# Nico59000/Ternary-image-codec

Measured on AMD Instinct MI355X. Metric: Mpix/s encode+decode 8K RS(26,20), higher is better.
Workload: dtype u8

## Files before the change

include/t3hip.h:

```cpp
#ifndef T3HIP_H
#define T3HIP_H

#include <stddef.h>
#include <stdint.h>

#ifdef __cplusplus
extern "C" {
#endif

#define T3_OK            0
#define T3_E_NODEVICE   -1
#define T3_E_HIP        -2
#define T3_E_ARG        -3
#define T3_E_CAPACITY   -4
#define T3_E_HEADER     -5
#define T3_E_RS         -6
#define T3_E_COMM       -7

#define T3_P1_RS26_24     0
#define T3_P2_RS26_22     1
#define T3_P3_RS26_20     2
#define T3_P4_RS26_18     3
#define T3_P5_RS26_22_2D  4
#define T3_RAW_MODE       0xFF
// ... 37 lines not shown
typedef struct t3_frame_record {
    uint64_t frame_idx;
    uint64_t n_words;
    uint64_t byte_offset;
    uint32_t crc32;
    uint32_t sym_sum;
    uint8_t  header_syms[54];
    uint8_t  profile;
    uint8_t  mode;
    uint8_t  pad_[8];
} t3_frame_record;

typedef struct t3hip_ctx t3hip_ctx;
int         t3hip_device_count(void);
int         t3hip_init(int device);
int         t3hip_shutdown(void);
int         t3hip_is_ready(void);
int         t3hip_create(int device, t3hip_ctx** out);
int         t3hip_destroy(t3hip_ctx* ctx);
int         t3hip_use(t3hip_ctx* ctx);
t3hip_ctx*  t3hip_current(void);
int         t3hip_ctx_device(const t3hip_ctx* ctx);
const char* t3hip_strerror(int code);
const char* t3hip_last_hip_error(void);
const char* t3hip_version(void);

void t3hip_cfg_default(t3_cfg* cfg);
int  t3hip_plan(uint64_t n_raw_words, const t3_cfg* cfg, t3_layout* out);
uint64_t t3hip_encoded_words(uint64_t n_raw_words, const t3_cfg* cfg);
int  t3hip_gf27_tables(uint8_t* exp78, int16_t* log27, uint8_t* mul729, uint8_t* inv27);
int  t3hip_rs_generator(int k, uint8_t* g_out);
int  t3hip_rs_parity_matrix(int k, int mode, uint8_t* P_out);
int  t3hip_mfma_encode_tables(int k, int mode, uint32_t* afrag768, uint32_t* lds_img3168);
int  t3hip_header_pack(const t3_cfg* cfg, uint32_t frame_seq, uint32_t band_map_hash, uint8_t syms27[27]);
int  t3hip_header_check(const uint8_t syms27[27]);
int  t3hip_header_unpack(const uint8_t syms27[27], t3_cfg* out, uint32_t* frame_seq, uint32_t* band_map_hash);
int  t3hip_header_encode(const t3_cfg* cfg, uint64_t n_raw_words, uint8_t* syms_out, uint32_t* n_syms);

int t3hip_pack_pixels(const void* px6, uint64_t n_px, void* words9);
int t3hip_unpack_words(const void* words9, uint64_t n_words, void* px6);
int t3hip_encode_profile(const void* raw9, uint64_t n_raw, const t3_cfg* cfg,
                         void* out9, uint64_t cap_words, uint64_t* n_out);
int t3hip_decode_profile(const void* in9, uint64_t n_in, t3_cfg* seen,
                         void* out9, uint64_t cap_words, uint64_t* n_out);
int t3hip_encode_frame(const void* px6, uint64_t n_px, const t3_cfg* cfg,
                       void* out9, uint64_t cap_words, uint64_t* n_out);
int t3hip_decode_frame(const void* in9, uint64_t n_in, t3_cfg* seen,
                       void* px6, uint64_t cap_px, uint64_t* n_px);

int t3hip_pack_pixels_dev(const void* d_px6, uint64_t n_px, void* d_words9, void* stream);
int t3hip_unpack_words_dev(const void* d_words9, uint64_t n_words, void* d_px6, void* stream);
int t3hip_encode_profile_dev(const void* d_raw9, uint64_t n_raw, const t3_cfg* cfg,
                             void* d_out9, uint64_t cap_words, uint64_t* n_out, void* stream);
int t3hip_encode_frame_dev(const void* d_px6, uint64_t n_px, const t3_cfg* cfg,
                           void* d_out9, uint64_t cap_words, uint64_t* n_out, void* stream);
int t3hip_decode_profile_dev(const void* d_in9, uint64_t n_in, t3_cfg* seen,
                             void* d_out, uint64_t cap_units, uint64_t* n_out,
                             int to_pixels, void* stream);
int t3hip_read_header_dev(const void* d_in9, uint64_t n_in, int mode, t3_cfg* out_cfg,
                          uint64_t* n_raw_words, void* stream);
int t3hip_decode_body_dev(const void* d_in9, uint64_t n_in, const t3_cfg* cfg, uint64_t n_raw_words,
                          void* d_out, uint64_t cap_units, uint64_t* n_out, int to_pixels,
                          uint32_t* d_fail, void* stream);

int t3hip_decode_frame_async(const void* d_in9, uint64_t n_in, const t3_cfg* cfg, uint64_t n_raw_words,
                             void* d_out, uint64_t cap_units, uint64_t* n_out, int to_pixels,
// ... 112 lines not shown
```

ternary-image-codec_amd/csrc/t3_api.cpp:

```cpp
#include <hip/hip_runtime.h>
#include <math.h>
#include <stdio.h>
#include <stdlib.h>
#include <string.h>

#include <algorithm>
#include <atomic>
#include <map>
#include <mutex>
#include <string>
#include <system_error>
#include <thread>
#include <tuple>
#include <vector>

#include "../../include/t3hip.h"
#include "t3_ctx.hpp"
#include "t3_host.hpp"
#include "t3_kernels.h"
#include "t3_decode.h"

using namespace t3;

namespace {
// ... 504 lines not shown
int t3hip_is_ready(void) { return ctx().ready ? 1 : 0; }
const char* t3hip_strerror(int c) {
    switch (c) {
        case T3_OK: return "ok"; case T3_E_NODEVICE: return "no usable gfx950 device (t3hip_init not done or failed)";
        case T3_E_HIP: return "HIP runtime error"; case T3_E_ARG: return "bad argument"; case T3_E_CAPACITY: return "output buffer too small";
        case T3_E_HEADER: return "superframe header did not decode (RS/CRC-12)"; case T3_E_RS: return "uncorrectable RS block";
        case T3_E_COMM: return "RCCL unavailable or collective failed";
    }
    return "unknown";
}
const char* t3hip_last_hip_error(void) { return ctx().hip_err.c_str(); }
const char* t3hip_version(void) { return "t3hip 0.1 (gfx950)"; }

void t3hip_cfg_default(t3_cfg* c) {
    memset(c, 0, sizeof *c);
    c->profile = T3_P2_RS26_22; for (int b = 0; b < 9; ++b) c->band_profile[b] = 1;
    c->seed_a = c->seed_b = c->seed_s0 = 1; c->superframe_words = 8192; c->subword = 27; c->centered = 1;
}
int t3hip_plan(uint64_t n_raw, const t3_cfg* cfg, t3_layout* out) { if (!cfg || !out) return T3_E_ARG; return plan(n_raw, *cfg, *out); }
uint64_t t3hip_encoded_words(uint64_t n_raw, const t3_cfg* cfg) { t3_layout L; if (!cfg || plan(n_raw, *cfg, L) != T3_OK) return 0; return L.out_words; }
int t3hip_gf27_tables(uint8_t* e78, int16_t* l27, uint8_t* m729, uint8_t* i27) {
    const Field& F = field();
    if (e78) memcpy(e78, F.exp78, 78); if (l27) memcpy(l27, F.log, sizeof F.log);
    if (m729) memcpy(m729, F.t.mul, 729); if (i27) memcpy(i27, F.t.inv, 27);
    return T3_OK;
}
int t3hip_rs_generator(int k, uint8_t* g_out) { if (!valid_k(k) || !g_out) return T3_E_ARG; rs_generator(k, g_out); return T3_OK; }
int t3hip_mfma_encode_tables(int k, int mode, uint32_t* afrag, uint32_t* lds_img) {
    if (!valid_k(k) || !afrag || !lds_img || mode < 0 || mode > 1) return T3_E_ARG;
    std::vector<uint32_t> a, l; build_mfma_encode(k, mode, a, l);
    memcpy(afrag, a.data(), a.size() * 4); memcpy(lds_img, l.data(), l.size() * 4);
    return T3_OK;
}
int t3hip_rs_parity_matrix(int k, int mode, uint8_t* P) { if (!valid_k(k) || !P || mode < 0 || mode > 1) return T3_E_ARG; rs_parity_matrix(k, mode, P); return T3_OK; }
int t3hip_header_pack(const t3_cfg* c, uint32_t fs, uint32_t bh, uint8_t s[27]) { if (!c || !s) return T3_E_ARG; header_pack(*c, fs, bh, s); return T3_OK; }
int t3hip_header_check(const uint8_t s[27]) { return s && header_check(s) ? 1 : 0; }
int t3hip_header_unpack(const uint8_t s[27], t3_cfg* o, uint32_t* fs, uint32_t* bh) { if (!s || !o) return T3_E_ARG; header_unpack(s, *o, fs, bh); return T3_OK; }
int t3hip_header_encode(const t3_cfg* c, uint64_t n_raw, uint8_t* out, uint32_t* n) {
    if (!c || !out || !n) return T3_E_ARG;
    t3_layout L; int rc = plan(n_raw, *c, L); if (rc) return rc;
    if (c->profile == T3_RAW_MODE) { *n = 0; return T3_OK; }
    *n = (uint32_t)header_encode(*c, n_raw, out); return T3_OK;
}

int t3hip_pack_pixels_dev(const void* d_px, uint64_t n_px, void* d_words, void* stream) {
    if (!ctx().ready) return T3_E_NODEVICE;
    const uint64_t nw = (n_px + 1) / 2; if (!nw) return T3_OK;
    if (!d_px || !d_words) return T3_E_ARG;
    hipLaunchKernelGGL(pack_pixels_kernel, dim3((unsigned)(((nw + 3) / 4 + 255) / 256)), dim3(256), 0, (hipStream_t)stream, (const uint16_t*)d_px, n_px, (uint8_t*)d_words, nw);
    HIPCHK(hipGetLastError()); return T3_OK;
}
int t3hip_unpack_words_dev(const void* d_words, uint64_t n_words, void* d_px, void* stream) {
    if (!ctx().ready) return T3_E_NODEVICE;
    if (!n_words) return T3_OK;
    if (!d_px || !d_words) return T3_E_ARG;
    hipLaunchKernelGGL(unpack_words_kernel, dim3((unsigned)(((n_words + 3) / 4 + 255) / 256)), dim3(256), 0, (hipStream_t)stream, (const uint8_t*)d_words, n_words, (uint16_t*)d_px);
    HIPCHK(hipGetLastError()); return T3_OK;
}
int t3hip_encode_profile_dev(const void* d_raw, uint64_t n_raw, const t3_cfg* cfg, void* d_out, uint64_t cap, uint64_t* n_out, void* stream) {
    return encode_dev(FE_WORDS, d_raw, n_raw, cfg, d_out, cap, n_out, (hipStream_t)stream);
}
int t3hip_encode_frame_dev(const void* d_px, uint64_t n_px, const t3_cfg* cfg, void* d_out, uint64_t cap, uint64_t* n_out, void* stream) {
    return encode_dev(FE_PIXELS, d_px, n_px, cfg, d_out, cap, n_out, (hipStream_t)stream);
}
int t3hip_rs_encode_blocks_dev(int k, int mode, const uint8_t* d_data, uint64_t n_blocks, uint8_t* d_code, void* stream) {
    Ctx& c = ctx(); if (!c.ready) return T3_E_NODEVICE;
// ... 177 lines not shown
```

ternary-image-codec_amd/csrc/t3_api_decode.cpp:

```cpp
#include <hip/hip_runtime.h>
#include <math.h>
#include <stdio.h>
#include <string.h>

#include <stdlib.h>

#include <algorithm>
#include <mutex>
#include <vector>

#include "../../include/t3hip.h"
#include "t3_ctx.hpp"
#include "t3_decode.h"
#include "t3_host.hpp"
#include "t3_window.h"

using namespace t3;

namespace {
struct HdrCheck { HdrExpect ex; uint32_t hs; uint32_t* verdict; const uint8_t* in; };

int launch_hdr_compare(const HdrCheck* h, hipStream_t s) {
    if (!h) return T3_OK;
    hipLaunchKernelGGL(hdr_compare_kernel, dim3(1), dim3(128), 0, s, h->in, h->ex, h->hs, h->verdict);
// ... 80 lines not shown
struct FusedPlan { DecFx2Args a; const void* fn; uint32_t grid, threads; bool tickets, whole_frame; };
int plan_fixed_fused(uint64_t body_bytes, uint32_t hdr_syms, const t3_layout& L, const ScrCycle& sc, void* d_out, uint64_t units, int to_pixels,
                     uint32_t* d_fail, FusedPlan& p, uint32_t bcn_slot = 0, uint32_t bcn_period = 0, uint32_t tile_lo = 0, uint32_t tile_hi = 0xFFFFFFFFu) {
    if (L.interleave2d || L.n_raw_words == 0) return 1;
    Ctx& c = ctx(); const DecodeTables& tab = c.dec;
    std::lock_guard<std::mutex> lk(c.tab_mu);
    if (!single_k(L)) return 1;
    const int k = L.band_k[0], ki = k_index(k);
    { const int rc = ensure_fx_tables(c.dec, k); if (rc) return rc; }
    DecFx2Args& a = p.a; memset(&a, 0, sizeof a);
    a.in_bytes = body_bytes; a.out = d_out; a.n_units = units; a.fail = d_fail; a.roots = tab.roots[ki];
    a.ttab = (to_pixels && T3_DEC_PX_TCOP == 16) ? tab.synd_T16 : tab.synd_T; a.small = tab.fx2_small; a.afrag = tab.synd_afrag[ki];
    const bool rgb = to_pixels == 2;
    if (rgb) { const int rc = rgb_dequant_tables(c, &a.dq); if (rc) return rc; }
    a.k = (uint32_t)k; a.nb = to_pixels ? (uint32_t)T3_DEC_PX_NB : 52u; a.div_nb = to_dev(fastdiv(a.nb)); a.TS = 9u * a.nb * (uint32_t)k; a.n_sym = (uint32_t)L.n_sym; a.hdr_syms = hdr_syms;
    const uint64_t maxb = *std::max_element(L.band_blocks, L.band_blocks + 9);
    a.n_tiles = (uint32_t)((maxb + a.nb - 1) / a.nb);
    fill_bands(a, L, (uint64_t)tile_lo * a.nb);
    if (tile_lo || tile_hi < a.n_tiles) {
        if (!to_pixels || bcn_period || tile_lo >= std::min(tile_hi, a.n_tiles)) return T3_E_ARG;
        const uint64_t u0 = (uint64_t)tile_lo * ((a.TS / 13u) * 3u);
        a.n_tiles = std::min(tile_hi, a.n_tiles) - tile_lo;
        a.out = (uint8_t*)d_out + u0 * (to_pixels == 2 ? 3u : 6u); a.n_units = units > u0 ? units - u0 : 0;
    }
    a.cyc24 = sc.cyc24; a.pre0 = sc.pre[0]; a.pre1 = sc.pre[1];
    scrambler_rows(a, sc);
    const bool bcn = bcn_period != 0;
    if (bcn) { a.bcn_slot = bcn_slot; a.bcn_pb = 9u * bcn_period - 1u; a.bcn_div = to_dev(fastdiv(a.bcn_pb)); }
    a.fma = tab.fma;
    const uint32_t ybytes = (a.TS + 16u + 15u) & ~15u;
    if (to_pixels) {
        a.fma_off = (uint32_t)kFx2TPx + 3u * 27u * 4u * (uint32_t)T3_DEC_PX_TCOP;
        a.af_off = a.fma_off + 19696u;
        a.pat_off = a.af_off + 3328u;
        a.y_off = a.pat_off + 192u; a.y_stride = ybytes;
        a.q_off = a.y_off + 2u * ybytes; a.q_stride = 10u * (uint32_t)kFx2QCap;
        a.o_off = a.q_off + 2u * a.q_stride; a.dq_off = a.o_off;
        a.lds_bytes = a.o_off + (rgb ? 336u : 16u);
    } else {
        a.fma_off = (uint32_t)kFx2TSeq + 3u * 27u * 4u * 32u;
        a.af_off = a.fma_off + 19696u;
        a.pat_off = a.af_off + 3328u;
        a.y_off = a.pat_off + 192u; a.y_stride = 0;
        a.q_off = a.y_off + ybytes; a.q_stride = 0;
        a.o_off = a.q_off + 10u * 512u;
        a.lds_bytes = a.o_off + (a.TS / 26u) * 27u + 64u;
    }
    const void* fn = nullptr;
    switch (26 - k) {
#define T3_PICKB(R, B) (rgb ? (const void*)decode_fixed_px_kernel<R, true, B> : to_pixels ? (const void*)decode_fixed_px_kernel<R, false, B> : (const void*)decode_fixed_kernel<R, B>)
#define T3_PICK(R) (bcn ? T3_PICKB(R, true) : T3_PICKB(R, false))
        case 2: fn = T3_PICK(2); break;
        case 4: fn = T3_PICK(4); break;
        case 6: fn = T3_PICK(6); break;
        default: fn = T3_PICK(8); break;
#undef T3_PICK
#undef T3_PICKB
    }
    p.fn = fn; p.threads = to_pixels ? T3_DEC_PX_THREADS : 512; p.tickets = to_pixels != 0; p.whole_frame = tile_lo == 0 && tile_hi == 0xFFFFFFFFu;
    return resident_grid(c, fn, (int)p.threads, a.lds_bytes, a.n_tiles, true, &p.grid);
}
int launch_fixed_fused(FusedPlan& p, const uint8_t* body, const HdrCheck* hdr, hipStream_t s) {
    Ctx& c = ctx(); DecFx2Args& a = p.a; const uint32_t grid = p.grid;
    a.in = body;
#ifdef T3_DEC_STAMPS
    static uint64_t* d_dbg = nullptr; static int calls = 0;
    if (!d_dbg) HIPCHK(hipMalloc((void**)&d_dbg, 16 * 8 * 4096));
    HIPCHK(hipMemsetAsync(d_dbg, 0, 16 * 8 * 4096, s));
    a.dbg = d_dbg;
#endif
    if (p.tickets) tile_tickets(c, s, 1, grid, &a.tile_ctr, &a.n_classes);
    { const int rc = settle_header(a, hdr, p.whole_frame, s); if (rc) return rc; }
    void* args[] = {(void*)&a};
    HIPCHK(hipLaunchKernel(p.fn, dim3(grid), dim3(p.threads), args, a.lds_bytes, s));
#ifdef T3_DEC_STAMPS
// ... 12 lines not shown
        fprintf(stderr, "[t3 dec stamps]   prologue (kernel entry -> first tile's input landed, wave 0): mean %.0f cycles/WG\n", acc[4] / grid);
        fprintf(stderr, "[t3 dec stamps]   timeline (us from first loop start): last start=%.1f last end=%.1f  workgroups starting >10 us late=%d\n", (s1 - s0) * 0.01, (e1 - s0) * 0.01, late);
    }
#endif
    return T3_OK;
}

struct UepPlan { DecUepArgs a; const void* fn; uint32_t grid; };
int plan_fixed_uep(uint64_t body_bytes, uint32_t hdr_syms, const t3_cfg& cfg, const t3_layout& L, const ScrCycle& sc,
                   void* d_out, uint64_t units, uint32_t* d_fail, UepPlan& p) {
    if (L.n_raw_words == 0 || L.n_sym + (1u << 20) >= (1ull << 32) || body_bytes + hdr_syms >= (1ull << 32)) return 1;
    if (getenv("T3HIP_TWO_KERNEL_DECODE") != nullptr) return 1;
    if (body_bytes >= (1ull << 28)) return 1;
    const bool il = L.interleave2d != 0 && cfg.tile_w > 1;
    DecUepArgs& a = p.a; memset(&a, 0, sizeof a);
    int gk[kUepMaxGrp]; uint32_t gn[kUepMaxGrp];
    const int ng = group_bands(a, L, gk, gn);
    if (!ng) return 1;
    if (ng == 2 && gk[0] > gk[1]) {
        std::swap(gk[0], gk[1]); std::swap(gn[0], gn[1]);
        uint8_t t[12]; memcpy(t, a.grp[0].bands, 12); memcpy(a.grp[0].bands, a.grp[1].bands, 12); memcpy(a.grp[1].bands, t, 12);
    }
    if (il) {
        const uint64_t A = (uint64_t)cfg.tile_w * cfg.tile_h;
        if (cfg.tile_w % 4u || (A % 4u && A < L.n_sym)) return 1;
        a.il_on = 1; a.il_w = cfg.tile_w; a.il_A = (uint32_t)std::min<uint64_t>(A, L.n_sym);
        if (a.il_A < 2 || a.il_w < 2) return 1;
        a.div_A = to_dev(fastdiv(a.il_A)); a.div_w = to_dev(fastdiv(a.il_w));
    }
    Ctx& c = ctx(); const DecodeTables& tab = c.dec;
    std::lock_guard<std::mutex> lk(c.tab_mu);
    uint32_t lcm = 1;
    for (int g = 0; g < ng; ++g) { const int rc = ensure_fx_tables(c.dec, gk[g]); if (rc) return rc; lcm = (uint32_t)lcm64(lcm, (uint32_t)gk[g]); }
    const uint32_t fixed_bytes = (uint32_t)kFx2TPx + 3u * 27u * 4u * 16u + 19696u + 3328u + 192u + 128u;
    const uint32_t budget = kLdsThreeWgs;
    uint32_t best_m = 0;
    for (uint32_t m = 1; 9u * lcm * m <= 12000u; ++m) {
        const uint32_t Lq = lcm * m, TS = 9u * Lq;
        if (TS % 4u) continue;
        uint32_t pairs = 0; bool small = false;
        for (int g = 0; g < ng; ++g) { const uint32_t nbg = Lq / (uint32_t)gk[g], items = gn[g] * nbg; if (nbg < 2u) small = true; if (nbg >= 2048u) pairs = 99; pairs += ((items + 31u) / 32u + 1u) / 2u; }
        if (small) continue;
        if (pairs > 8u) break;
        const uint32_t ybytes = (TS + 16u + 15u) & ~15u;
        if (fixed_bytes + 2u * ybytes + 2u * 10u * 96u + 64u > budget) break;
        best_m = m;
    }
    if (!best_m) return 1;
    const uint32_t Lq = lcm * best_m;
    a.TS = 9u * Lq; a.n_sym = (uint32_t)L.n_sym; a.hdr_syms = hdr_syms; a.n_grp = (uint32_t)ng;
    a.in_bytes = body_bytes; a.out = d_out; a.n_units = units; a.fail = d_fail;
    a.ttab = tab.synd_T16; a.small = tab.fx2_small; a.fma = tab.fma;
    a.fma_off = (uint32_t)kFx2TPx + 3u * 27u * 4u * 16u;
    uint32_t off = a.fma_off + 19696u;
    uint64_t tiles = 0; uint32_t items_all = 0;
    for (int g = 0; g < ng; ++g) {
        auto& G = a.grp[g]; const int ki = k_index(gk[g]);
        G.r = 26u - (uint32_t)gk[g]; G.nb = Lq / (uint32_t)gk[g]; G.n_items = gn[g] * G.nb; G.div_nb = to_dev(fastdiv(G.nb));
        G.afrag = tab.synd_afrag[ki]; G.roots = tab.roots[ki];
        if (g == 0) { G.af_off = off; off += 3328u; } else G.af_off = a.grp[0].af_off;
        items_all += G.n_items;
        for (uint32_t i = 0; i < gn[g]; ++i) tiles = std::max<uint64_t>(tiles, (L.band_blocks[G.bands[i]] + G.nb - 1) / G.nb);
    }
    a.n_tiles = (uint32_t)tiles;
    a.pat_off = off; off += 192u; a.rec_off = off; off += 128u;
    const uint32_t ybytes = (a.TS + 16u + 15u) & ~15u;
    a.y_off = off; a.y_stride = ybytes; off += 2u * ybytes;
    const uint32_t q_entries = std::min<uint32_t>((budget - 64u - off) / 20u, items_all);
    uint32_t qrel = 0;
    for (int g = 0; g < ng; ++g) { auto& G = a.grp[g]; G.q_cap = std::max<uint32_t>(8u, (uint32_t)((uint64_t)q_entries * G.n_items / items_all) & ~3u); G.q_rel = qrel; qrel += 10u * G.q_cap; }
    a.q_off = off; a.q_stride = (qrel + 15u) & ~15u; off += 2u * a.q_stride;
    a.lds_bytes = off + 16u;
    if (a.lds_bytes > 160u * 1024u) return 1;
    {
        for (int i = 0; i < 8; ++i) a.pair_tab[i] = 0xFFFFFFFFu;
        uint32_t p = 0;
        for (int g = 0; g < ng; ++g) for (uint32_t it0 = 0; it0 < a.grp[g].n_items; it0 += 64u, ++p) a.pair_tab[2u * (p % 4u) + p / 4u] = (uint32_t)g | it0 << 8;
    }
    fill_bands(a, L);
    scrambler_rows(a, sc);
    const void* fn = nullptr;
    {
        const int ra = 26 - gk[0], rb = ng == 2 ? 26 - gk[1] : ra;
#define T3_UEP(A, B) if (ra == A && rb == B) fn = (const void*)decode_uep_px_kernel<A, B>;
        T3_UEP(2, 2) T3_UEP(4, 4) T3_UEP(6, 6) T3_UEP(8, 8) T3_UEP(4, 2) T3_UEP(6, 2) T3_UEP(6, 4) T3_UEP(8, 2) T3_UEP(8, 4) T3_UEP(8, 6)
#undef T3_UEP
        if (!fn) return 1;
    }
    p.fn = fn;
    return resident_grid(c, fn, 512, a.lds_bytes, a.n_tiles, true, &p.grid);
}
int launch_fixed_uep(UepPlan& p, const uint8_t* body, const HdrCheck* hdr, hipStream_t s) {
    Ctx& c = ctx(); DecUepArgs& a = p.a;
// ... 385 lines not shown
```

ternary-image-codec_amd/csrc/t3_decode_fx2.h:

```cpp
#pragma once
#include "t3_decode_fx.h"
#include "t3_host.hpp"

namespace t3 {
namespace {

__device__ __forceinline__ uint32_t mod26(uint32_t u) { return min(u, u + 26u); }

struct Synd { uint32_t lo, hi; };

typedef uint32_t Geo;
struct Blk { bool valid, first; uint32_t c0, off, yb; };
constexpr uint32_t kFx2Dummy = 384;

template <int R>
__device__ __forceinline__ Geo fx2_geo(const uint32_t item, const uint32_t n_items, const uint32_t nb, const DevDiv& div_nb, const uint32_t tile0, uint32_t& off0) {
    constexpr uint32_t K = 26 - R;
    const uint32_t bi = min(div_ge2(item, div_nb), 8u), m = item - bi * nb;
    const uint32_t m3 = m - 3u * ((m * 683u) >> 11);
    const Row rw = row(bi);
    uint32_t cb = rw.boff6 + 2u * m3; cb -= cb >= 6u ? 6u : 0u;
    off0 = (uint32_t)rw.body_off + 26u * (tile0 * nb + m);
    return (bi + 9u * K * m) | cb << 16 | (item < n_items ? 1u << 19 : 0u);
}
template <int R>
__device__ __forceinline__ bool fx2_has_block(const Geo g, const uint32_t tile, const uint32_t n_tiles, const uint32_t nb) {
    constexpr uint32_t K = 26 - R;
    bool v = (g >> 19) != 0u;
    if (tile + 1u >= n_tiles) {
        const uint32_t yr = g & 0xFFFFu, m = yr / (9u * K), bi = yr - 9u * K * m;
        v = v && tile * nb + m < row(bi).blocks;
    }
    return v;
}
__device__ __forceinline__ Blk fx2_block(const Geo g, const uint32_t off, const bool valid, const uint32_t u2, const uint32_t y_off) {
    Blk b;
    b.valid = valid;
    b.first = off == 0u;
    b.c0 = ((g >> 16) & 7u) + u2;
    b.off = off;
    b.yb = y_off + (g & 0xFFFFu);
    return b;
}

template <int R, uint32_t TCOP, uint32_t TBASE, uint32_t MT, uint32_t SMB = 0, int RM = R>
__device__ __forceinline__ Synd fx2_set(const Blk& b, const uint32_t (&Lw)[4], const uint32_t lane, const uint32_t af_off, const uint32_t pat_off) {
    constexpr uint32_t mt = MT;
    constexpr uint32_t K = 26 - R, H = RM / 2, HB = R / 2;
    static_assert(RM >= R, "matrix of the code with more parity");
    const uint32_t n = lane & 31u, h = lane >> 5;
    uint32_t W[4];
#pragma unroll
    for (int i = 0; i < 3; ++i) W[i] = __builtin_amdgcn_alignbyte(Lw[i + 1], Lw[i], 3u * h);
    W[3] = Lw[3] >> (24u * h);
    uint32_t hi = (W[3] | (W[3] + 0x65u)) & 0x80u;
#pragma unroll
    for (int i = 0; i < 3; ++i) hi |= (W[i] | (W[i] + 0x65656565u)) & 0x80808080u;
    if (__builtin_amdgcn_ballot_w64(b.valid && hi != 0u) != 0) {
#pragma unroll
        for (int i = 0; i < 4; ++i) {
            uint32_t r = 0;
#pragma unroll
            for (int q = 0; q < 4; ++q) { const uint32_t c = (W[i] >> (8 * q)) & 0xFFu; r |= (c - 27u * div27(c)) << (8 * q); }
            W[i] = r;
        }
    }
    const uint32_t prow = (b.first && h == 0u) ? 11u : b.c0 + h;
    const v4i P = *T3_LDS(const v4i, pat_off + 16u * prow);
#pragma unroll
    for (int i = 0; i < 4; ++i) W[i] += (uint32_t)P[i];
    const uint32_t tb0 = 4u * (n % TCOP);
    const uint32_t ya = b.valid ? b.yb + 117u * h : SMB + kFx2Dummy;
    v16i acc = {64, 64, 64, 64, 64, 64, 64, 64, 64, 64, 64, 64, 64, 64, 64, 64};
    auto fetch = [&](const uint32_t st, v4i& Bv) {
        Bv = v4i{0, 0, 0, 0};
#pragma unroll
        for (uint32_t d = 0; d < 4; ++d) {
            const uint32_t q = 4u * st + d;
            if (q >= 13u) continue;
            const uint32_t c = __builtin_amdgcn_ubfe(W[st], 8u * d, 8u);
            Bv[d] = (int)*T3_LDS(const uint32_t, TBASE + ((c * (4u * TCOP)) | tb0));
        }
    };
    auto emit = [&](const uint32_t st, const v4i& Bv) {
#pragma unroll
        for (uint32_t d = 0; d < 4; ++d) { const uint32_t q = 4u * st + d; if (q < 13u && q + 13u < K) *T3_LDS(uint8_t, ya + 9u * q) = (uint8_t)((uint32_t)Bv[d] >> 16); }
        if (4u * st + 3u + 13u >= K) {
            if (h == 0) {
#pragma unroll
                for (uint32_t d = 0; d < 4; ++d) { const uint32_t q = 4u * st + d; if (q < 13u && q + 13u >= K) *T3_LDS(uint8_t, ya + 9u * q) = (uint8_t)((uint32_t)Bv[d] >> 16); }
            }
        }
    };
    v4i Bq[2];
    fetch(0, Bq[0]);
#pragma unroll
    for (uint32_t st = 0; st < 4; ++st) {
        if (st < 3u) fetch(st + 1u, Bq[(st + 1u) & 1u]);
        v4i Af = {0, 0, 0, 0};
        if (st < 3u) Af = *T3_LDS(const v4i, af_off + 16u * (64u * st + lane)); else Af[0] = *T3_LDS(const int, af_off + 3072u + 4u * lane);
        emit(st, Bq[st & 1u]);
        acc = __builtin_amdgcn_mfma_i32_32x32x32_i8(Af, Bq[st & 1u], acc, 0, 0, 0);
        __builtin_amdgcn_sched_barrier(0);
    }
    uint32_t Pown = 0;
#pragma unroll
    for (uint32_t jj = 0; jj < H; ++jj) {
        const uint32_t s = lds_u8(mt + 14u + (uint32_t)acc[3 * jj]) + lds_u8(mt + 174u + (uint32_t)acc[3 * jj + 1]) + lds_u8(mt + 334u + (uint32_t)acc[3 * jj + 2]);
        Pown |= s << (8u * jj);
    }
    const auto sw = __builtin_amdgcn_permlane32_swap(Pown, Pown, false, false);
    Synd r; r.lo = sw[0]; r.hi = sw[1];
    if constexpr (RM != R) {
        const uint64_t V = (uint64_t)sw[0] | (uint64_t)sw[1] << (8u * H);
        constexpr uint64_t M = (1ull << (8u * HB)) - 1ull;
        r.lo = (uint32_t)(V & M); r.hi = (uint32_t)((V >> (8u * HB)) & M);
    }
    return r;
}

template <int R, uint32_t SMB = 0>
__device__ __forceinline__ uint32_t fx2_single(const Synd& sy, const uint32_t yb, const uint32_t FMA) {
    constexpr uint32_t SM = SMB + kFx2Small;
    constexpr uint32_t K = 26 - R, H = R / 2;
    uint32_t lg[R]; bool ok = true;
#pragma unroll
    for (uint32_t j = 0; j < (uint32_t)R; ++j) {
        const uint32_t s = ((j < H ? sy.lo : sy.hi) >> (8u * (j % H))) & 0xFFu;
        lg[j] = lds_u8(SM + kFx2LG + s);
        ok = ok && lg[j] != 0xFFu;
    }
    const uint32_t p = mod26(lg[1] - lg[0]);
#pragma unroll
    for (uint32_t j = 1; j + 1 < (uint32_t)R; ++j) ok = ok && mod26(lg[j + 1] - lg[j]) == p;
// ... 15 lines not shown
#pragma unroll
    for (int j = 0; j < R; ++j) Sx[j] = __umul24(S[j], 729u) + FMA;
    uint32_t sg[T + 1], sg27[T + 1], bs27[T + 1];
#pragma unroll
    for (int i = 0; i <= T; ++i) { sg[i] = 0; sg27[i] = 0; bs27[i] = 0; }
    sg[0] = 1; sg27[0] = 27; bs27[1] = 27u * 2u;
    uint32_t L = 0;
    bool over = false;
#pragma unroll
    for (int n = 0; n < R; ++n) {
        uint32_t d = S[n];
#pragma unroll
        for (int i = 1; i <= T; ++i) if (i <= n) d = tab(Sx[n - i] + sg27[i] + d);
        const bool upd = d != 0 && 2u * L <= (uint32_t)n;
        const uint32_t dx = __umul24(d, 729u) + FMA;
        uint32_t old27[T + 1];
#pragma unroll
        for (int i = 0; i <= T; ++i) old27[i] = sg27[i];
#pragma unroll
        for (int i = 1; i <= T; ++i) if (i <= n + 1) { sg[i] = tab(dx + bs27[i] + sg[i]); sg27[i] = 27u * sg[i]; }
        const uint32_t ninv = lds_u8(SM + kFx2NINV + d), nix = __umul24(ninv, 729u) + FMA;
        uint32_t nb27[T + 1];
        nb27[0] = 0; nb27[1] = 27u * ninv;
#pragma unroll
        for (int i = 2; i <= T; ++i) nb27[i] = (i <= n + 1) ? 27u * tab(nix + old27[i - 1]) : 0u;
        if (upd) { L = (uint32_t)n + 1u - L; over = over || L > (uint32_t)T; }
#pragma unroll
        for (int i = T; i >= 1; --i) bs27[i] = upd ? nb27[i] : bs27[i - 1];
        bs27[0] = 0;
    }
    uint32_t deg = 0;
#pragma unroll
    for (int i = 1; i <= T; ++i) if (sg[i] != 0) deg = (uint32_t)i;
    if (over || deg != L) return 1u;
    uint32_t ridx = sg[T];
#pragma unroll
    for (int q = T - 1; q >= 1; --q) ridx = ridx * 27u + sg[q];
    const uint32_t roots = root_tbl[ridx];
    const uint32_t np = (uint32_t)__popc(roots);
    if (np != deg) return 1u;
    uint32_t Om[T];
#pragma unroll
    for (int q = 0; q < T; ++q) {
        uint32_t acc = S[q];
#pragma unroll
        for (int j = 1; j <= q; ++j) acc = tab(Sx[q - j] + sg27[j] + acc);
        Om[q] = acc;
    }
    uint32_t s22 = 0;
    if constexpr (T >= 2) s22 = tab(FMA + 729u + sg27[2] + sg[2]);
    const uint32_t s22_27 = 27u * s22;
    if constexpr (WIDE) {
        uint32_t r = roots, bad = 0u;
        uint32_t pe[T], xix[T];
    #pragma unroll
        for (int e = 0; e < T; ++e) {
            const bool have = (uint32_t)e < np;
            const uint32_t p = have ? (uint32_t)__ffs((int)r) - 1u : 0u; r &= r - 1u;
            pe[e] = p;
            xix[e] = __umul24(lds_u8(SM + kFx2EX + (p == 0 ? 0u : 26u - p)), 729u) + FMA;
        }
        uint32_t num[T], den[T];
    #pragma unroll
        for (int e = 0; e < T; ++e) { num[e] = Om[T - 1]; den[e] = tab(xix[e] + s22_27 + sg[1]); }
    #pragma unroll
        for (int q = T - 2; q >= 0; --q) {
    #pragma unroll
            for (int e = 0; e < T; ++e) num[e] = tab(xix[e] + 27u * num[e] + Om[q]);
        }
        if constexpr (T >= 4) {
    #pragma unroll
            for (int e = 0; e < T; ++e) { const uint32_t x2 = tab(xix[e] + sg27[4]); const uint32_t x3 = tab(xix[e] + 27u * x2); den[e] = tab(xix[e] + 27u * x3 + den[e]); }
        }
    #pragma unroll
        for (int e = 0; e < T; ++e) {
            const bool have = (uint32_t)e < np;
            bad |= (have && den[e] == 0u) ? 1u : 0u;
            fx.pos[e] = pe[e]; fx.mag[e] = tab(FMA + 729u * lds_u8(SM + kFx2NEG + num[e]) + 27u * lds_u8(SM + kFx2INV + den[e]));
        }
        if (bad) return 1u;
    } else {
        uint32_t r = roots;
#pragma unroll
        for (int e = 0; e < T; ++e) {
// ... 77 lines not shown
```

ternary-image-codec_amd/csrc/t3_decode_wg.h:

```cpp
#pragma once
#include "t3_decode_fx.h"
#include "t3_host.hpp"

namespace t3 {
namespace {

template <class A>
__device__ __forceinline__ void stage_band_rows(const A& a) {
#pragma unroll
    for (int b = 0; b < 9; ++b) { Row r; r.blocks = a.band_blocks[b]; r.boff6 = a.band_boff6[b]; r.body_off = a.band_body_off[b]; *(Row*)(lds + 16 * b) = r; }
}

template <uint32_t TCOP, uint32_t TBASE, uint32_t MT, class A>
__device__ __forceinline__ void stage_fx2_tables(const A& a, const uint32_t* const& afrag, const uint32_t& af_off, const uint32_t tid, const uint32_t nthr) {
    for (uint32_t i = tid * 16u; i < (uint32_t)kFx2SmallBytes; i += nthr * 16u) *(uint4*)(lds + kFx2Small + i) = *(const uint4*)(a.small + i);
    for (uint32_t i = tid * 16u; i < (uint32_t)kFx2ModBytes; i += nthr * 16u) *(uint4*)(lds + MT + i) = *(const uint4*)(a.small + kFx2SmallBytes + i);
    for (uint32_t i = tid * 16u; i < 3u * 27u * 4u * TCOP; i += nthr * 16u) *(uint4*)(lds + TBASE + i) = *(const uint4*)((const uint8_t*)a.ttab + i);
    for (uint32_t i = tid * 16u; i < 19696u; i += nthr * 16u) *(uint4*)(lds + a.fma_off + i) = *(const uint4*)(a.fma + i);
    for (uint32_t i = tid * 16u; i < 3072u; i += nthr * 16u) *(uint4*)(lds + af_off + i) = *(const uint4*)((const uint8_t*)afrag + i);
    if (tid < 64u) *(uint32_t*)(lds + af_off + 3072u + 4u * tid) = afrag[(3u * 64u + tid) * 4u];
}
template <class A>
__device__ __forceinline__ void stage_pattern_rows(const A& a, const uint32_t tid) {
    if (tid == 64u) {
#pragma unroll
        for (int i = 0; i < 48; ++i) *(uint32_t*)(lds + a.pat_off + 4 * i) = a.pat[i];
    }
}

struct Tickets {
    bool dyn; uint32_t grid, NC, cls, wgc; uint32_t* ctr;
    __device__ __forceinline__ void first(const uint32_t tid) const { if (tid == 0) *(uint32_t*)(lds + kFx2Next + 4u) = dyn ? cls + NC * (wgc + atomicAdd(ctr, 1u)) : blockIdx.x + grid; }
    __device__ __forceinline__ uint32_t request() const { return atomicAdd(ctr, 1u); }
    __device__ __forceinline__ void publish(const uint32_t buf, const uint32_t& raw, const uint32_t& nxt) const {
        *(uint32_t*)(lds + kFx2Next + 4u * buf) = dyn ? cls + NC * (wgc + raw) : nxt + grid;
    }
    __device__ __forceinline__ uint32_t next(const uint32_t buf) const { return __builtin_amdgcn_readfirstlane(*(const uint32_t*)(lds + kFx2Next + 4u * buf)); }
    template <class A>
    __device__ __forceinline__ void finish(const A& a, const uint32_t tid) const {
        if (dyn && tid == 0u) {
            if (a.verdict) { const uint32_t wgf = *(const uint32_t*)(lds + kFx2FailWg); if (wgf) atomicAdd(a.fail, wgf); }
            asm volatile("s_waitcnt vmcnt(0)" ::: "memory");
            if (atomicAdd(a.tile_ctr + 64u * NC, 1u) == grid - 1u) {
                if (a.verdict) a.verdict[1] = atomicExch(a.fail, 0u);
                for (uint32_t c = 0; c <= NC; ++c) __hip_atomic_store(a.tile_ctr + 64u * c, 0u, __ATOMIC_RELAXED, __HIP_MEMORY_SCOPE_AGENT);
            }
        }
    }
};
template <class A>
__device__ __forceinline__ Tickets tickets_setup(const A& a) {
    Tickets t;
    t.grid = gridDim.x; t.dyn = a.tile_ctr != nullptr;
// ... 44 lines not shown
```

ternary-image-codec_amd/csrc/t3_host.cpp:

```cpp
#include "t3_host.hpp"

#include <string.h>

namespace t3 {

namespace {
struct V3 { int t[3]; };
V3 to_v(int s) { return V3{{s % 3, (s / 3) % 3, (s / 9) % 3}}; }
int to_s(const V3& v) { return v.t[0] + 3 * v.t[1] + 9 * v.t[2]; }
int mul_poly(int a, int b) {
    V3 x = to_v(a), y = to_v(b);
    int c[5] = {0, 0, 0, 0, 0};
    for (int i = 0; i < 3; ++i) for (int j = 0; j < 3; ++j) c[i + j] += x.t[i] * y.t[j];
    c[2] += c[4]; c[1] += 2 * c[4];
    c[1] += c[3]; c[0] += 2 * c[3];
    return (c[0] % 3) + 3 * (c[1] % 3) + 9 * (c[2] % 3);
}
Field make_field() {
    Field f; memset(&f, 0, sizeof f);
    for (int a = 0; a < 27; ++a) {
        V3 x = to_v(a);
        for (int b = 0; b < 27; ++b) {
            V3 y = to_v(b);
            f.t.add[a * 27 + b] = (uint8_t)to_s(V3{{(x.t[0] + y.t[0]) % 3, (x.t[1] + y.t[1]) % 3, (x.t[2] + y.t[2]) % 3}});
// ... 167 lines not shown

void mfma_scrambler_table(int k, const ScrCycle& sc, uint32_t out[12]) {
    const int r = 26 - k;
    for (int c = 0; c < 6; ++c) {
        uint32_t dw[2] = {0, 0};
        for (int j = 0; j < r && j < 8; ++j) dw[j / 4] |= (uint32_t)sc.cyc[(c + j) % 6] << (8 * (j % 4));
        out[2 * c] = dw[0]; out[2 * c + 1] = dw[1];
    }
}

int syndrome_lut_slab(int k) { return 26 - k == 8 ? 768 : 512; }
void build_syndrome_lut(int k, std::vector<uint32_t>& image) {
    const Field& F = field(); RsView v = rs_view(F.t);
    const int r = 26 - k, nmain = r < 5 ? r : 5, slab = syndrome_lut_slab(k);
    image.assign((size_t)26 * slab / 4, 0u);
    for (int i = 0; i < 26; ++i) {
        uint32_t* sl = image.data() + (size_t)i * slab / 4;
        for (int c = 0; c < 27; ++c) {
            uint32_t dw[6] = {0, 0, 0, 0, 0, 0};
            for (int j = 0; j < r; ++j) {
                const int y = v.M((uint8_t)c, v.P((j + 1) * i));
                const int tr[3] = {y % 3, (y / 3) % 3, y / 9};
                if (j < nmain) for (int q = 0; q < 3; ++q) dw[q] |= (uint32_t)tr[q] << (6 * j);
                else for (int q = 0; q < 3; ++q) { const int f = 3 * (j - 5) + q; dw[3 + f / 5] |= (uint32_t)tr[q] << (6 * (f % 5)); }
            }
            for (int q = 0; q < (r == 8 ? 5 : 4); ++q) sl[32 * q + c] = dw[q];
        }
    }
}

void build_mfma_syndrome(int k, std::vector<uint32_t>& afrag) {
    const Field& F = field(); RsView v = rs_view(F.t);
    const int r = 26 - k, H = r / 2;
    afrag.assign(4 * 64 * 4, 0u);
    for (int s = 0; s < 4; ++s) for (int l = 0; l < 64; ++l) for (int d = 0; d < 4; ++d) {
        const int m = l & 31, kh = l >> 5, hh = (m >> 2) & 1, i = (m & 3) + 4 * (m >> 3);
        const int q = 4 * s + d;
        if (q >= 13 || i >= 3 * H) continue;
        const int p = 13 * kh + q, j = hh * H + i / 3, t = i % 3;
        const uint8_t g = v.P((j + 1) * p);
        uint32_t dw = 0;
        for (int tt = 0; tt < 3; ++tt) {
            const int e = tt == 0 ? 1 : tt == 1 ? 3 : 9;
            const int c = F.t.mul[e * 27 + g];
            const int tr[3] = {c % 3, (c / 3) % 3, c / 9};
            dw |= (uint32_t)(tr[t] == 2 ? 0xFFu : (uint32_t)tr[t]) << (tt == 2 ? 24 : 8 * tt);
        }
        afrag[(size_t)(s * 64 + l) * 4 + d] = dw;
    }
}
void build_syndrome_T(std::vector<uint32_t>& img, int copies) {
    const Field& F = field();
    img.assign((size_t)3 * 27 * copies, 0u);
    auto sb = [](int t) { return (uint32_t)(t == 2 ? 0xFF : t); };
    for (int st = 0; st < 3; ++st) for (int c = 0; c < 27; ++c) {
        const int d = F.t.add[c * 27 + F.t.neg[13 * st]];
        const uint32_t dw = sb(d % 3) | sb((d / 3) % 3) << 8 | (uint32_t)d << 16 | sb(d / 9) << 24;
        for (int b = 0; b < copies; ++b) img[((size_t)st * 27 + c) * copies + b] = dw;
    }
}
void build_fx2_small(uint8_t out[kFx2SmallBytes]) {
    const Field& F = field();
    memset(out, 0, kFx2SmallBytes);
    for (int x = 0; x < 27; ++x) {
        out[kFx2LG + x] = x ? (uint8_t)F.log[x] : 0xFF;
        out[kFx2INV + x] = F.t.inv[x]; out[kFx2NEG + x] = F.t.neg[x]; out[kFx2NINV + x] = F.t.neg[F.t.inv[x]];
    }
    for (int i = 0; i < 26; ++i) out[kFx2EX + i] = F.t.exp[i];
}
void build_fx2_mod(uint8_t out[kFx2ModBytes]) {
    for (int t = 0; t < 3; ++t) for (int x = 0; x < 160; ++x) out[160 * t + x] = (uint8_t)((((x - 78) % 3 + 3) % 3) * (t == 0 ? 1 : t == 1 ? 3 : 9));
}

ScrCycle scrambler_cycle_from_next(const uint8_t next[3], uint32_t s0) {
    ScrCycle c; memset(&c, 0, sizeof c);
    for (int i = 0; i < 3; ++i) c.next[i] = next[i];
    uint32_t st = s0 % 3; uint8_t seq[8];
    for (int i = 0; i < 8; ++i) { st = next[st]; seq[i] = (uint8_t)st; }
    c.pre[0] = seq[0]; c.pre[1] = seq[1];
    for (int i = 0; i < 6; ++i) c.cyc[i] = seq[2 + i];
// ... 210 lines not shown
```

Before: 127,100.

## Fold 13th syndrome symbol into spare MFMA lanes, cutting one MFMA step

The RS syndrome computation previously used four MFMA i8 steps, the last of which handled only symbol 12. Its coefficients are now packed into the unused byte slot of the first three A-fragment entries. The matching B entry is spliced in with perm, so syndromes take three MFMAs, and the LDS A-fragment table drops from 3328 to 3072 bytes. The high-bit check is also reordered and the Chien/degree early-exit checks are moved later to shorten the dependency chain. The change relies on the packed layout staying bit-exact with the host table builder.

```diff
diff --git a/include/t3hip.h b/include/t3hip.h
--- a/include/t3hip.h
+++ b/include/t3hip.h
@@ -93,6 +93,7 @@
 int  t3hip_rs_generator(int k, uint8_t* g_out);
 int  t3hip_rs_parity_matrix(int k, int mode, uint8_t* P_out);
 int  t3hip_mfma_encode_tables(int k, int mode, uint32_t* afrag768, uint32_t* lds_img3168);
+int  t3hip_mfma_syndrome_tables(int k, uint32_t* afrag768);
 int  t3hip_header_pack(const t3_cfg* cfg, uint32_t frame_seq, uint32_t band_map_hash, uint8_t syms27[27]);
 int  t3hip_header_check(const uint8_t syms27[27]);
 int  t3hip_header_unpack(const uint8_t syms27[27], t3_cfg* out, uint32_t* frame_seq, uint32_t* band_map_hash);
diff --git a/ternary-image-codec_amd/csrc/t3_api.cpp b/ternary-image-codec_amd/csrc/t3_api.cpp
--- a/ternary-image-codec_amd/csrc/t3_api.cpp
+++ b/ternary-image-codec_amd/csrc/t3_api.cpp
@@ -560,6 +560,12 @@
     memcpy(afrag, a.data(), a.size() * 4); memcpy(lds_img, l.data(), l.size() * 4);
     return T3_OK;
 }
+int t3hip_mfma_syndrome_tables(int k, uint32_t* afrag) {
+    if (!valid_k(k) || !afrag) return T3_E_ARG;
+    std::vector<uint32_t> a; build_mfma_syndrome(k, a);
+    memcpy(afrag, a.data(), a.size() * 4);
+    return T3_OK;
+}
 int t3hip_rs_parity_matrix(int k, int mode, uint8_t* P) { if (!valid_k(k) || !P || mode < 0 || mode > 1) return T3_E_ARG; rs_parity_matrix(k, mode, P); return T3_OK; }
 int t3hip_header_pack(const t3_cfg* c, uint32_t fs, uint32_t bh, uint8_t s[27]) { if (!c || !s) return T3_E_ARG; header_pack(*c, fs, bh, s); return T3_OK; }
 int t3hip_header_check(const uint8_t s[27]) { return s && header_check(s) ? 1 : 0; }
diff --git a/ternary-image-codec_amd/csrc/t3_api_decode.cpp b/ternary-image-codec_amd/csrc/t3_api_decode.cpp
--- a/ternary-image-codec_amd/csrc/t3_api_decode.cpp
+++ b/ternary-image-codec_amd/csrc/t3_api_decode.cpp
@@ -136,7 +136,7 @@
     if (to_pixels) {
         a.fma_off = (uint32_t)kFx2TPx + 3u * 27u * 4u * (uint32_t)T3_DEC_PX_TCOP;
         a.af_off = a.fma_off + 19696u;
-        a.pat_off = a.af_off + 3328u;
+        a.pat_off = a.af_off + 3072u;
         a.y_off = a.pat_off + 192u; a.y_stride = ybytes;
         a.q_off = a.y_off + 2u * ybytes; a.q_stride = 10u * (uint32_t)kFx2QCap;
         a.o_off = a.q_off + 2u * a.q_stride; a.dq_off = a.o_off;
@@ -144,7 +144,7 @@
     } else {
         a.fma_off = (uint32_t)kFx2TSeq + 3u * 27u * 4u * 32u;
         a.af_off = a.fma_off + 19696u;
-        a.pat_off = a.af_off + 3328u;
+        a.pat_off = a.af_off + 3072u;
         a.y_off = a.pat_off + 192u; a.y_stride = 0;
         a.q_off = a.y_off + ybytes; a.q_stride = 0;
         a.o_off = a.q_off + 10u * 512u;
@@ -223,7 +223,7 @@
     std::lock_guard<std::mutex> lk(c.tab_mu);
     uint32_t lcm = 1;
     for (int g = 0; g < ng; ++g) { const int rc = ensure_fx_tables(c.dec, gk[g]); if (rc) return rc; lcm = (uint32_t)lcm64(lcm, (uint32_t)gk[g]); }
-    const uint32_t fixed_bytes = (uint32_t)kFx2TPx + 3u * 27u * 4u * 16u + 19696u + 3328u + 192u + 128u;
+    const uint32_t fixed_bytes = (uint32_t)kFx2TPx + 3u * 27u * 4u * 16u + 19696u + 3072u + 192u + 128u;
     const uint32_t budget = kLdsThreeWgs;
     uint32_t best_m = 0;
     for (uint32_t m = 1; 9u * lcm * m <= 12000u; ++m) {
@@ -249,7 +249,7 @@
         auto& G = a.grp[g]; const int ki = k_index(gk[g]);
         G.r = 26u - (uint32_t)gk[g]; G.nb = Lq / (uint32_t)gk[g]; G.n_items = gn[g] * G.nb; G.div_nb = to_dev(fastdiv(G.nb));
         G.afrag = tab.synd_afrag[ki]; G.roots = tab.roots[ki];
-        if (g == 0) { G.af_off = off; off += 3328u; } else G.af_off = a.grp[0].af_off;
+        if (g == 0) { G.af_off = off; off += 3072u; } else G.af_off = a.grp[0].af_off;
         items_all += G.n_items;
         for (uint32_t i = 0; i < gn[g]; ++i) tiles = std::max<uint64_t>(tiles, (L.band_blocks[G.bands[i]] + G.nb - 1) / G.nb);
     }
diff --git a/ternary-image-codec_amd/csrc/t3_decode_fx2.h b/ternary-image-codec_amd/csrc/t3_decode_fx2.h
--- a/ternary-image-codec_amd/csrc/t3_decode_fx2.h
+++ b/ternary-image-codec_amd/csrc/t3_decode_fx2.h
@@ -53,9 +53,10 @@
 #pragma unroll
     for (int i = 0; i < 3; ++i) W[i] = __builtin_amdgcn_alignbyte(Lw[i + 1], Lw[i], 3u * h);
     W[3] = Lw[3] >> (24u * h);
-    uint32_t hi = (W[3] | (W[3] + 0x65u)) & 0x80u;
-#pragma unroll
-    for (int i = 0; i < 3; ++i) hi |= (W[i] | (W[i] + 0x65656565u)) & 0x80808080u;
+    uint32_t hi = W[0] | (W[0] + 0x65656565u);
+#pragma unroll
+    for (int i = 1; i < 3; ++i) hi |= W[i] | (W[i] + 0x65656565u);
+    hi = (hi & 0x80808080u) | ((W[3] | (W[3] + 0x65u)) & 0x80u);
     if (__builtin_amdgcn_ballot_w64(b.valid && hi != 0u) != 0) {
 #pragma unroll
         for (int i = 0; i < 4; ++i) {
@@ -72,34 +73,38 @@
     const uint32_t tb0 = 4u * (n % TCOP);
     const uint32_t ya = b.valid ? b.yb + 117u * h : SMB + kFx2Dummy;
     v16i acc = {64, 64, 64, 64, 64, 64, 64, 64, 64, 64, 64, 64, 64, 64, 64, 64};
+    auto entry = [&](const uint32_t q) -> uint32_t {
+        const uint32_t c = __builtin_amdgcn_ubfe(W[q / 4u], 8u * (q % 4u), 8u);
+        return *T3_LDS(const uint32_t, TBASE + ((c * (4u * TCOP)) | tb0));
+    };
     auto fetch = [&](const uint32_t st, v4i& Bv) {
-        Bv = v4i{0, 0, 0, 0};
-#pragma unroll
-        for (uint32_t d = 0; d < 4; ++d) {
-            const uint32_t q = 4u * st + d;
-            if (q >= 13u) continue;
-            const uint32_t c = __builtin_amdgcn_ubfe(W[st], 8u * d, 8u);
-            Bv[d] = (int)*T3_LDS(const uint32_t, TBASE + ((c * (4u * TCOP)) | tb0));
-        }
+#pragma unroll
+        for (uint32_t d = 0; d < 4; ++d) Bv[d] = (int)entry(4u * st + d);
     };
     auto emit = [&](const uint32_t st, const v4i& Bv) {
 #pragma unroll
-        for (uint32_t d = 0; d < 4; ++d) { const uint32_t q = 4u * st + d; if (q < 13u && q + 13u < K) *T3_LDS(uint8_t, ya + 9u * q) = (uint8_t)((uint32_t)Bv[d] >> 16); }
+        for (uint32_t d = 0; d < 4; ++d) { const uint32_t q = 4u * st + d; if (q + 13u < K) *T3_LDS(uint8_t, ya + 9u * q) = (uint8_t)((uint32_t)Bv[d] >> 16); }
         if (4u * st + 3u + 13u >= K) {
             if (h == 0) {
 #pragma unroll
-                for (uint32_t d = 0; d < 4; ++d) { const uint32_t q = 4u * st + d; if (q < 13u && q + 13u >= K) *T3_LDS(uint8_t, ya + 9u * q) = (uint8_t)((uint32_t)Bv[d] >> 16); }
+                for (uint32_t d = 0; d < 4; ++d) { const uint32_t q = 4u * st + d; if (q + 13u >= K) *T3_LDS(uint8_t, ya + 9u * q) = (uint8_t)((uint32_t)Bv[d] >> 16); }
             }
         }
     };
     v4i Bq[2];
     fetch(0, Bq[0]);
-#pragma unroll
-    for (uint32_t st = 0; st < 4; ++st) {
-        if (st < 3u) fetch(st + 1u, Bq[(st + 1u) & 1u]);
-        v4i Af = {0, 0, 0, 0};
-        if (st < 3u) Af = *T3_LDS(const v4i, af_off + 16u * (64u * st + lane)); else Af[0] = *T3_LDS(const int, af_off + 3072u + 4u * lane);
+    const uint32_t E12 = entry(12u);
+#pragma unroll
+    for (uint32_t st = 0; st < 3; ++st) {
+        if (st < 2u) fetch(st + 1u, Bq[(st + 1u) & 1u]);
+        const v4i Af = *T3_LDS(const v4i, af_off + 16u * (64u * st + lane));
         emit(st, Bq[st & 1u]);
+        if (st == 0u) {
+            if (h == 0) *T3_LDS(uint8_t, ya + 9u * 12u) = (uint8_t)(E12 >> 16);
+            Bq[0][0] = (int)__builtin_amdgcn_perm(E12, (uint32_t)Bq[0][0], 0x03040100u);
+            Bq[0][1] = (int)__builtin_amdgcn_perm(E12, (uint32_t)Bq[0][1], 0x03050100u);
+            Bq[0][2] = (int)__builtin_amdgcn_perm(E12, (uint32_t)Bq[0][2], 0x03070100u);
+        }
         acc = __builtin_amdgcn_mfma_i32_32x32x32_i8(Af, Bq[st & 1u], acc, 0, 0, 0);
         __builtin_amdgcn_sched_barrier(0);
     }
@@ -181,13 +186,10 @@
     uint32_t deg = 0;
 #pragma unroll
     for (int i = 1; i <= T; ++i) if (sg[i] != 0) deg = (uint32_t)i;
-    if (over || deg != L) return 1u;
     uint32_t ridx = sg[T];
 #pragma unroll
     for (int q = T - 1; q >= 1; --q) ridx = ridx * 27u + sg[q];
     const uint32_t roots = root_tbl[ridx];
-    const uint32_t np = (uint32_t)__popc(roots);
-    if (np != deg) return 1u;
     uint32_t Om[T];
 #pragma unroll
     for (int q = 0; q < T; ++q) {
@@ -198,7 +200,12 @@
     }
     uint32_t s22 = 0;
     if constexpr (T >= 2) s22 = tab(FMA + 729u + sg27[2] + sg[2]);
+#pragma unroll
+    for (int q = 0; q < T; ++q) asm volatile("" : "+v"(Om[q]));
+    asm volatile("" : "+v"(s22));
     const uint32_t s22_27 = 27u * s22;
+    const uint32_t np = (uint32_t)__popc(roots);
+    if (over || deg != L || np != deg) return 1u;
     if constexpr (WIDE) {
         uint32_t r = roots, bad = 0u;
         uint32_t pe[T], xix[T];
diff --git a/ternary-image-codec_amd/csrc/t3_decode_wg.h b/ternary-image-codec_amd/csrc/t3_decode_wg.h
--- a/ternary-image-codec_amd/csrc/t3_decode_wg.h
+++ b/ternary-image-codec_amd/csrc/t3_decode_wg.h
@@ -18,7 +18,6 @@
     for (uint32_t i = tid * 16u; i < 3u * 27u * 4u * TCOP; i += nthr * 16u) *(uint4*)(lds + TBASE + i) = *(const uint4*)((const uint8_t*)a.ttab + i);
     for (uint32_t i = tid * 16u; i < 19696u; i += nthr * 16u) *(uint4*)(lds + a.fma_off + i) = *(const uint4*)(a.fma + i);
     for (uint32_t i = tid * 16u; i < 3072u; i += nthr * 16u) *(uint4*)(lds + af_off + i) = *(const uint4*)((const uint8_t*)afrag + i);
-    if (tid < 64u) *(uint32_t*)(lds + af_off + 3072u + 4u * tid) = afrag[(3u * 64u + tid) * 4u];
 }
 template <class A>
 __device__ __forceinline__ void stage_pattern_rows(const A& a, const uint32_t tid) {
diff --git a/ternary-image-codec_amd/csrc/t3_host.cpp b/ternary-image-codec_amd/csrc/t3_host.cpp
--- a/ternary-image-codec_amd/csrc/t3_host.cpp
+++ b/ternary-image-codec_amd/csrc/t3_host.cpp
@@ -223,20 +223,20 @@
 void build_mfma_syndrome(int k, std::vector<uint32_t>& afrag) {
     const Field& F = field(); RsView v = rs_view(F.t);
     const int r = 26 - k, H = r / 2;
-    afrag.assign(4 * 64 * 4, 0u);
-    for (int s = 0; s < 4; ++s) for (int l = 0; l < 64; ++l) for (int d = 0; d < 4; ++d) {
+    afrag.assign(3 * 64 * 4, 0u);
+    auto coef = [&](int p, int j, int tt, int t) -> uint32_t {
+        const int e = tt == 0 ? 1 : tt == 1 ? 3 : 9;
+        const int c = F.t.mul[e * 27 + v.P((j + 1) * p)];
+        const int tr[3] = {c % 3, (c / 3) % 3, c / 9};
+        return tr[t] == 2 ? 0xFFu : (uint32_t)tr[t];
+    };
+    for (int s = 0; s < 3; ++s) for (int l = 0; l < 64; ++l) for (int d = 0; d < 4; ++d) {
         const int m = l & 31, kh = l >> 5, hh = (m >> 2) & 1, i = (m & 3) + 4 * (m >> 3);
-        const int q = 4 * s + d;
-        if (q >= 13 || i >= 3 * H) continue;
-        const int p = 13 * kh + q, j = hh * H + i / 3, t = i % 3;
-        const uint8_t g = v.P((j + 1) * p);
+        if (i >= 3 * H) continue;
+        const int p = 13 * kh + 4 * s + d, j = hh * H + i / 3, t = i % 3;
         uint32_t dw = 0;
-        for (int tt = 0; tt < 3; ++tt) {
-            const int e = tt == 0 ? 1 : tt == 1 ? 3 : 9;
-            const int c = F.t.mul[e * 27 + g];
-            const int tr[3] = {c % 3, (c / 3) % 3, c / 9};
-            dw |= (uint32_t)(tr[t] == 2 ? 0xFFu : (uint32_t)tr[t]) << (tt == 2 ? 24 : 8 * tt);
-        }
+        for (int tt = 0; tt < 3; ++tt) dw |= coef(p, j, tt, t) << (tt == 2 ? 24 : 8 * tt);
+        if (s == 0 && d < 3) dw |= coef(13 * kh + 12, j, d, t) << 16;
         afrag[(size_t)(s * 64 + l) * 4 + d] = dw;
     }
 }
```

Result: no change. 127,600, median of 5 (+0.4%).
